# UT-Austin-RPL/FORGE

Measured on AMD Instinct MI355X. Metric: rendered views/sec (5 views, 128^2 px, 64^3 voxel), higher is better.
Workload: dtype f32; 1 GPU; BASELINE configs[1]: FORGE hot path, 1 scene(s)/GPU x 5 input views 256^2 -> 32^3x128 feature grid -> 64^3 render grid -> 5 views x 128^2 rays x 64 samples -> 5 RGB 256^2; HIP rotate, fp32-MFMA implicit-GEMM ResNet-50 trunk / conv1 / ConvGRU (Winograd F(2x2,3x3) x 3 depth taps) / heads / conv_rgb, HIP ray-march (no MIOpen/rocBLAS kernel in the step); eval BN, random-init seeded weights; scenes_per_gpu=1, views_in=5, views_out=5, feature_grid=32, render_grid=64, steps_in_flight=4, launch=hipGraph replay, 4 steps in flight on 4 HIP streams, parallelism=dp1 (scene-sharded, no data-path collective; 4-scalar RCC...

## Files before the change

### forge_amd/csrc/winograd.hip

```cpp
#include "common.h"

namespace forge {

__device__ __forceinline__ float4 add(float4 a, float4 b) { return make_float4(a.x + b.x, a.y + b.y, a.z + b.z, a.w + b.w); }
__device__ __forceinline__ float4 sub(float4 a, float4 b) { return make_float4(a.x - b.x, a.y - b.y, a.z - b.z, a.w - b.w); }
__device__ __forceinline__ float add(float a, float b) { return a + b; }
__device__ __forceinline__ float sub(float a, float b) { return a - b; }
__device__ __forceinline__ float4 fma4(float k, float4 a, float4 b) { return make_float4(fmaf(k, a.x, b.x), fmaf(k, a.y, b.y), fmaf(k, a.z, b.z), fmaf(k, a.w, b.w)); }

__device__ __forceinline__ void f43_six_lines(float p0, float p1, float p2, float p3, float p4, float p5, float& q0, float& q1, float& q2, float& q3, float& q4,
                                              float& q5) {
    const float a02 = p0 - p2, a24 = p2 - p4, s34 = p3 + p4, s12 = p1 + p2, d43 = p4 - p3, d12 = p1 - p2;
    const float d42 = p4 - p2, d31 = p3 - p1, d13 = p1 - p3, d35 = p3 - p5;
    q0 = fmaf(4.f, a02, -a24);
    q1 = fmaf(-4.f, s12, s34);
    q2 = fmaf(4.f, d12, d43);
    q3 = fmaf(2.f, d31, d42);
    q4 = fmaf(-2.f, d31, d42);
    q5 = fmaf(4.f, d13, -d35);
}

__device__ __forceinline__ void tile_decode(long long idx, int per, int cs, int Ht, int Wt, unsigned& r, int& c, int& tw, int& th, unsigned& t) {
    r = (unsigned)(idx / per);
    c = (int)(idx - (long long)r * per) << cs;
    unsigned q = r;
    t = q / (unsigned)Wt;
    tw = (int)(q - t * (unsigned)Wt); q = t; t = q / (unsigned)Ht;
    th = (int)(q - t * (unsigned)Ht);
}

template <typename T>
__device__ __forceinline__ void bt_cols_store(const T (&w)[4], float* vp, int i, long long ptv) {
    *reinterpret_cast<T*>(vp + (4 * i + 0) * ptv) = sub(w[0], w[2]);
    *reinterpret_cast<T*>(vp + (4 * i + 1) * ptv) = add(w[1], w[2]);
    *reinterpret_cast<T*>(vp + (4 * i + 2) * ptv) = sub(w[2], w[1]);
    *reinterpret_cast<T*>(vp + (4 * i + 3) * ptv) = sub(w[1], w[3]);
}

template <typename T, typename I>
__device__ __forceinline__ void bt_d_b_store(const T (&d)[4][4], float* V, I row, int ld, int c, long long ptv) {
    T w[4][4];
#pragma unroll
    for (int j = 0; j < 4; ++j) {
        w[0][j] = sub(d[0][j], d[2][j]);
        w[1][j] = add(d[1][j], d[2][j]);
        w[2][j] = sub(d[2][j], d[1][j]);
        w[3][j] = sub(d[1][j], d[3][j]);
    }
    float* vp = V + (long long)row * ld + c;
#pragma unroll
    for (int i = 0; i < 4; ++i) bt_cols_store(w[i], vp, i, ptv);
}

__device__ __forceinline__ void a_y_at_store(float4 y00, float4 y01, float4 y10, float4 y11, float* mp, long long ptm) {
    const float4 zero = make_float4(0.f, 0.f, 0.f, 0.f);
    const float4 s[4][2] = {{y00, y01}, {add(y00, y10), add(y01, y11)}, {sub(y00, y10), sub(y01, y11)}, {sub(zero, y10), sub(zero, y11)}};
#pragma unroll
    for (int i = 0; i < 4; ++i) {
        *reinterpret_cast<float4*>(mp + (4 * i + 0) * ptm) = s[i][0];
        *reinterpret_cast<float4*>(mp + (4 * i + 1) * ptm) = add(s[i][0], s[i][1]);
        *reinterpret_cast<float4*>(mp + (4 * i + 2) * ptm) = sub(s[i][0], s[i][1]);
        *reinterpret_cast<float4*>(mp + (4 * i + 3) * ptm) = sub(zero, s[i][1]);
    }
}

__device__ __forceinline__ double depth_row_f23(int k, double w0, double w1, double w2) {
    return k == 0 ? w0 : k == 1 ? 0.5 * (w0 + w1 + w2) : k == 2 ? 0.5 * (w0 - w1 + w2) : w2;
}
__device__ __forceinline__ double depth_row_f43(int k, double w0, double w1, double w2) {
    return k == 0 ? 0.25 * w0 : k == 1 ? -((w0 + w2) + w1) / 6.0 : k == 2 ? -((w0 + w2) - w1) / 6.0
         : k == 3 ? ((0.25 * w0 + w2) + 0.5 * w1) / 6.0 : k == 4 ? ((0.25 * w0 + w2) - 0.5 * w1) / 6.0 : w2;
}

template <int NH = 4, double (*HROW)(int, double, double, double) = depth_row_f23>
__device__ __forceinline__ void g_d_gt_store(const double (&d)[3][3], float* up, long long pt) {
    double g[NH][3];
#pragma unroll
    for (int b = 0; b < 3; ++b)
#pragma unroll
        for (int i = 0; i < NH; ++i) g[i][b] = HROW(i, d[0][b], d[1][b], d[2][b]);
#pragma unroll
    for (int i = 0; i < NH; ++i) {
        up[(4 * i + 0) * pt] = (float)g[i][0];
        up[(4 * i + 1) * pt] = (float)(0.5 * (g[i][0] + g[i][1] + g[i][2]));
        up[(4 * i + 2) * pt] = (float)(0.5 * (g[i][0] - g[i][1] + g[i][2]));
        up[(4 * i + 3) * pt] = (float)g[i][2];
    }
}

struct WinoInArgs {
    const float* in; int ld; long long bs;
    float* V; int ldv; long long ptv;
    int n, D, H, W, C;
    int nsum; long long ss;
    float* dM; long long ptm;
};

template <bool DY>
__global__ __launch_bounds__(256) void wino_input_kernel(const WinoInArgs a) {
    const int C4 = a.C >> 2, Ht = a.H >> 1, Wt = a.W >> 1;
    const long long idx = (long long)xcd_remap(blockIdx.x, gridDim.x) * 256 + threadIdx.x;
    const long long R = (long long)a.n * a.D * Ht * Wt;
    if (idx >= R * C4) return;
    unsigned r, t;
    int c, tw, th;
    tile_decode(idx, C4, 2, Ht, Wt, r, c, tw, th, t);
    const unsigned q = t; t = q / (unsigned)a.D;
    const int z = (int)(q - t * (unsigned)a.D);
    const float* base = a.in + ((long long)t * a.bs + (long long)z * a.H * a.W) * a.ld + c;
    float4 d[4][4];
#pragma unroll
    for (int i = 0; i < 4; ++i) {
        const int y = 2 * th - 1 + i;
#pragma unroll
        for (int j = 0; j < 4; ++j) {
            const int x = 2 * tw - 1 + j;
            const bool ok = (unsigned)y < (unsigned)a.H && (unsigned)x < (unsigned)a.W;
            float4 v = make_float4(0.f, 0.f, 0.f, 0.f);
            if (ok) {
                const float* p = base + ((long long)y * a.W + x) * a.ld;
                v = *reinterpret_cast<const float4*>(p);
                if (a.nsum > 1) {
                    for (int k = 1; k < a.nsum; ++k) v = add(v, *reinterpret_cast<const float4*>(p + (long long)k * a.ss * a.ld));
                    const float inv = 1.f / (float)a.nsum;
                    v = make_float4(v.x * inv, v.y * inv, v.z * inv, v.w * inv);
                }
            }
            d[i][j] = v;
        }
    }
    if constexpr (DY) a_y_at_store(d[1][1], d[1][2], d[2][1], d[2][2], a.dM + (long long)r * a.C + c, a.ptm);
    bt_d_b_store(d, a.V, r, a.ldv, c, a.ptv);
}

template <int TH>
__global__ __launch_bounds__(256) void wino_input_dn4_kernel(const WinoInArgs a) {
    constexpr int NR = TH + 2;
    const int Ht = TH == 4 ? a.H >> 2 : a.H >> 1, Wt = a.W >> 1, Dg = a.D >> 2;
    const long long idx = (long long)xcd_remap(blockIdx.x, gridDim.x) * 256 + threadIdx.x;
    const long long RG = (long long)a.n * Dg * Ht * Wt;
    if (idx >= RG * a.C) return;
    unsigned r, t;
    int c, tw, th;
    tile_decode(idx, a.C, 0, Ht, Wt, r, c, tw, th, t);
    const unsigned q = t; t = q / (unsigned)Dg;
    const int g = (int)(q - t * (unsigned)Dg);
    const long long HW = (long long)a.H * a.W;
    const float* base = a.in + (long long)t * a.bs * a.ld + c;
    const float inv = 1.f / (float)a.nsum;
    float d[6][NR][4];
#pragma unroll
    for (int i = 0; i < NR; ++i) {
        const int y = TH * th - 1 + i;
#pragma unroll
        for (int j = 0; j < 4; ++j) {
            const int x = 2 * tw - 1 + j;
            const bool ok = (unsigned)y < (unsigned)a.H && (unsigned)x < (unsigned)a.W;
            float p[6];
#pragma unroll
            for (int e = 0; e < 6; ++e) {
                const int z = 4 * g - 1 + e;
                float v = 0.f;
                if (ok && (unsigned)z < (unsigned)a.D) {
                    const float* s = base + ((long long)z * HW + (long long)y * a.W + x) * a.ld;
                    v = *s;
                    if (a.nsum > 1) {
                        for (int k = 1; k < a.nsum; ++k) v += s[(long long)k * a.ss * a.ld];
                        v *= inv;
                    }
                }
                p[e] = v;
            }
            f43_six_lines(p[0], p[1], p[2], p[3], p[4], p[5], d[0][i][j], d[1][i][j], d[2][i][j], d[3][i][j], d[4][i][j], d[5][i][j]);
        }
    }
    const long long HWt = (long long)Ht * Wt;
    float* vp = a.V + ((((long long)t * Dg + g) * 6) * HWt + (long long)th * Wt + tw) * a.ldv + c;
    if constexpr (TH == 4) {
#pragma unroll
        for (int k = 0; k < 6; ++k) {
#pragma unroll
            for (int j = 0; j < 4; ++j)
                f43_six_lines(d[k][0][j], d[k][1][j], d[k][2][j], d[k][3][j], d[k][4][j], d[k][5][j], d[k][0][j], d[k][1][j], d[k][2][j], d[k][3][j], d[k][4][j], d[k][5][j]);
#pragma unroll
            for (int i = 0; i < 6; ++i) bt_cols_store(d[k][i], vp + k * HWt * a.ldv, i, a.ptv);
        }
    } else {
#pragma unroll
        for (int k = 0; k < 6; ++k) bt_d_b_store(d[k], vp, k * HWt, a.ldv, 0, a.ptv);
    }
}

__global__ __launch_bounds__(256) void wino_weight_kernel(const float* __restrict__ wp, float* __restrict__ U, int Cout, int Cin, int KD, int transpose) {
    const int No = transpose ? Cin : Cout, Nc = transpose ? Cout : Cin;
    const long long idx = (long long)blockIdx.x * 256 + threadIdx.x, per = (long long)No * Nc;
    if (idx >= KD * per) return;
    const int kd = (int)(idx / per);
    const long long oc = idx - kd * per;
    const int o = (int)(oc / Nc), c = (int)(oc - (long long)o * Nc);
    double w[3][3];
#pragma unroll
    for (int a = 0; a < 3; ++a)
#pragma unroll
        for (int b = 0; b < 3; ++b) {
            const int tap = transpose ? ((KD - 1 - kd) * 3 + (2 - a)) * 3 + (2 - b) : (kd * 3 + a) * 3 + b;
            w[a][b] = (double)wp[((long long)tap * Cout + (transpose ? c : o)) * Cin + (transpose ? o : c)];
        }
    g_d_gt_store(w, U + ((long long)kd * No + o) * Nc + c, KD * per);
}

template <int K, double (*ROW)(int, double, double, double), int NH = 4, double (*HROW)(int, double, double, double) = depth_row_f23>
__global__ __launch_bounds__(256) void wino_weight_nest_kernel(const float* __restrict__ wp, float* __restrict__ U, int Cout, int Cin) {
    const long long idx = (long long)blockIdx.x * 256 + threadIdx.x, per = (long long)Cout * Cin;
    if (idx >= per) return;
    double w[3][3][3];
#pragma unroll
    for (int t = 0; t < 27; ++t) w[t / 9][(t / 3) % 3][t % 3] = (double)wp[t * per + idx];
#pragma unroll
    for (int k = 0; k < K; ++k) {
        double d[3][3];
#pragma unroll
        for (int a = 0; a < 3; ++a)
#pragma unroll
            for (int b = 0; b < 3; ++b) d[a][b] = ROW(k, w[0][a][b], w[1][a][b], w[2][a][b]);
        g_d_gt_store<NH, HROW>(d, U + k * per + idx, K * per);
    }
}

enum WinoEpilogue : int { W_BIAS = 0, W_AFFINE_ACT = 1, W_GRU_GATES = 2, W_GRU_OUT = 3 };

struct WinoOutArgs {
    const float* Mm; long long ptm;
    const float* Mm2; long long ptm2, bs2;
    const float* bias; const float* scale; const float* shift; float slope;
    const float* residual;
    const float* aux_h; const float* aux_z;
    float* out; float* out2; float* out3; int ldo;
    int n, D, H, W, Cout, epi;
};

template <int ROWS>
__device__ __forceinline__ void load_planes(float4 (&m)[ROWS][4], const float* Mm, long long ptm, const float* Mm2, long long ptm2, long long bs2, int Cout, unsigned R1, unsigned r, int c) {
    const float* mp = Mm + (long long)r * Cout + c;
#pragma unroll
    for (int i = 0; i < ROWS; ++i)
#pragma unroll
        for (int j = 0; j < 4; ++j) m[i][j] = *reinterpret_cast<const float4*>(mp + (4 * i + j) * ptm);
    if (Mm2) {
        const unsigned nn = r / R1;
        const float* mp2 = Mm2 + ((long long)nn * bs2 + (r - nn * R1)) * Cout + c;
#pragma unroll
        for (int i = 0; i < ROWS; ++i)
#pragma unroll
            for (int j = 0; j < 4; ++j) m[i][j] = add(m[i][j], *reinterpret_cast<const float4*>(mp2 + (4 * i + j) * ptm2));
    }
}

template <int EPI, bool HALF = false, int TH = 2>
__global__ __launch_bounds__(256) void wino_output_kernel(const WinoOutArgs a) {
    static_assert(TH == 2 || (TH == 4 && !HALF), "tiles of 2 x 2 voxels, or of 4 x 2 from the 24 points");
    const int C4 = a.Cout >> 2, Ht = TH == 4 ? a.H >> 2 : a.H >> 1, Wt = a.W >> 1;
    const long long idx = (long long)blockIdx.x * 256 + threadIdx.x;
    const long long R = (long long)a.n * a.D * Ht * Wt;
    if (idx >= R * C4) return;
    unsigned r, t;
    int c, tw, th;
    tile_decode(idx, C4, 2, Ht, Wt, r, c, tw, th, t);
    float4 s[TH][4];
    if constexpr (TH == 4) {
        const float* mp = a.Mm + (long long)r * a.Cout + c;
#pragma unroll
        for (int j = 0; j < 4; ++j) {
            float4 m[6];
#pragma unroll
            for (int i = 0; i < 6; ++i) m[i] = *reinterpret_cast<const float4*>(mp + (4 * i + j) * a.ptm);
            const float4 sl = add(m[1], m[2]), dl = sub(m[1], m[2]), Sl = add(m[3], m[4]), Dl = sub(m[3], m[4]);
            s[0][j] = add(add(sl, Sl), m[0]);
            s[1][j] = fma4(2.f, Dl, dl);
            s[2][j] = fma4(4.f, Sl, sl);
            s[3][j] = add(fma4(8.f, Dl, dl), m[5]);
        }
    } else if constexpr (HALF) {
        load_planes<2>(s, a.Mm, a.ptm, a.Mm2, a.ptm2, a.bs2, a.Cout, (unsigned)(a.D * Ht * Wt), r, c);
    } else {
        float4 m[4][4];
        load_planes<4>(m, a.Mm, a.ptm, a.Mm2, a.ptm2, a.bs2, a.Cout, (unsigned)(a.D * Ht * Wt), r, c);
#pragma unroll
        for (int j = 0; j < 4; ++j) {
            s[0][j] = add(add(m[0][j], m[1][j]), m[2][j]);
            s[1][j] = sub(sub(m[1][j], m[2][j]), m[3][j]);
        }
    }
    float4 y[TH][2];
#pragma unroll
    for (int i = 0; i < TH; ++i) {
        y[i][0] = add(add(s[i][0], s[i][1]), s[i][2]);
        y[i][1] = sub(sub(s[i][1], s[i][2]), s[i][3]);
    }
    float4 bias = make_float4(0.f, 0.f, 0.f, 0.f), sc = make_float4(1.f, 1.f, 1.f, 1.f), sh = bias;
    if (a.bias) bias = *reinterpret_cast<const float4*>(a.bias + c);
    if ((EPI == W_AFFINE_ACT || (EPI == W_GRU_OUT && a.out2)) && a.scale) {
        sc = *reinterpret_cast<const float4*>(a.scale + c);
        sh = *reinterpret_cast<const float4*>(a.shift + c);
    }
    const int Ch = a.Cout >> 1;
    const long long plane = (long long)t * a.H * a.W;
#pragma unroll
    for (int i = 0; i < TH; ++i)
#pragma unroll
        for (int j = 0; j < 2; ++j) {
            const long long orow = plane + (long long)(TH * th + i) * a.W + (2 * tw + j);
            float v[4] = {y[i][j].x + bias.x, y[i][j].y + bias.y, y[i][j].z + bias.z, y[i][j].w + bias.w};
            if (a.residual) {
                const float4 rr = *reinterpret_cast<const float4*>(a.residual + orow * a.Cout + c);
                v[0] += rr.x; v[1] += rr.y; v[2] += rr.z; v[3] += rr.w;
            }
            const float scv[4] = {sc.x, sc.y, sc.z, sc.w}, shv[4] = {sh.x, sh.y, sh.z, sh.w};
            if constexpr (EPI == W_BIAS) {
                *reinterpret_cast<float4*>(a.out + orow * a.ldo + c) = make_float4(v[0], v[1], v[2], v[3]);
            } else if constexpr (EPI == W_AFFINE_ACT) {
#pragma unroll
                for (int k = 0; k < 4; ++k) {
                    const float u = fmaf(v[k], scv[k], shv[k]);
                    v[k] = u > 0.f ? u : u * a.slope;
                }
                *reinterpret_cast<float4*>(a.out + orow * a.ldo + c) = make_float4(v[0], v[1], v[2], v[3]);
            } else if constexpr (EPI == W_GRU_GATES) {
                float g[4];
#pragma unroll
                for (int k = 0; k < 4; ++k) g[k] = 1.f / (1.f + expf(-v[k]));
                if (c < Ch) {
                    *reinterpret_cast<float4*>(a.out + orow * Ch + c) = make_float4(g[0], g[1], g[2], g[3]);
                } else {
                    const float4 h = *reinterpret_cast<const float4*>(a.aux_h + orow * Ch + (c - Ch));
                    *reinterpret_cast<float4*>(a.out2 + orow * Ch + (c - Ch)) = make_float4(h.x * g[0], h.y * g[1], h.z * g[2], h.w * g[3]);
                    if (a.out3) *reinterpret_cast<float4*>(a.out3 + orow * Ch + (c - Ch)) = make_float4(g[0], g[1], g[2], g[3]);
                }
            } else {
                const float4 z4 = *reinterpret_cast<const float4*>(a.aux_z + orow * a.Cout + c);
                const float4 h4 = *reinterpret_cast<const float4*>(a.aux_h + orow * a.Cout + c);
                const float zv[4] = {z4.x, z4.y, z4.z, z4.w}, hv[4] = {h4.x, h4.y, h4.z, h4.w};
                float cand[4], hn[4];
#pragma unroll
                for (int k = 0; k < 4; ++k) {
                    cand[k] = tanhf(v[k]);
                    hn[k] = hv[k] * (1.f - zv[k]) + cand[k] * zv[k];
                }
                *reinterpret_cast<float4*>(a.out + orow * a.ldo + c) = make_float4(hn[0], hn[1], hn[2], hn[3]);
                if (a.out2)
                    *reinterpret_cast<float4*>(a.out2 + orow * a.ldo + c) =
                        make_float4(fmaf(hn[0], scv[0], shv[0]), fmaf(hn[1], scv[1], shv[1]), fmaf(hn[2], scv[2], shv[2]), fmaf(hn[3], scv[3], shv[3]));
                if (a.out3) *reinterpret_cast<float4*>(a.out3 + orow * a.ldo + c) = make_float4(cand[0], cand[1], cand[2], cand[3]);
            }
        }
}

struct WinoDyArgs {
    const float* dy; int ldy;
    float* dM; long long ptm;
    int n, D, H, W, Cout;
};

__global__ __launch_bounds__(256) void wino_dy_kernel(const WinoDyArgs a) {
    const int C4 = a.Cout >> 2, Ht = a.H >> 1, Wt = a.W >> 1;
    const long long idx = (long long)blockIdx.x * 256 + threadIdx.x;
    const long long R = (long long)a.n * a.D * Ht * Wt;
    if (idx >= R * C4) return;
    unsigned r, t;
    int c, tw, th;
    tile_decode(idx, C4, 2, Ht, Wt, r, c, tw, th, t);
    const float* yp = a.dy + ((long long)t * a.H * a.W + (long long)(2 * th) * a.W + 2 * tw) * a.ldy + c;
    float4 y[2][2];
#pragma unroll
    for (int i = 0; i < 2; ++i)
#pragma unroll
        for (int j = 0; j < 2; ++j) y[i][j] = *reinterpret_cast<const float4*>(yp + ((long long)i * a.W + j) * a.ldy);
    a_y_at_store(y[0][0], y[0][1], y[1][0], y[1][1], a.dM + (long long)r * a.Cout + c, a.ptm);
}

__global__ __launch_bounds__(256) void wino_dw_kernel(const float* __restrict__ dU, float* __restrict__ dw, int Cout, int Cin, int KD) {
    const long long idx = (long long)blockIdx.x * 256 + threadIdx.x, per = (long long)Cout * Cin;
    if (idx >= KD * per) return;
    const int kd = (int)(idx / per);
    const long long oc = idx - kd * per;
    const long long pt = KD * per;
    float u[4][4];
#pragma unroll
    for (int i = 0; i < 4; ++i)
#pragma unroll
        for (int j = 0; j < 4; ++j) u[i][j] = dU[(4 * i + j) * pt + kd * per + oc];
    float g[3][4];
#pragma unroll
    for (int j = 0; j < 4; ++j) {
        g[0][j] = u[0][j] + 0.5f * (u[1][j] + u[2][j]);
        g[1][j] = 0.5f * (u[1][j] - u[2][j]);
        g[2][j] = 0.5f * (u[1][j] + u[2][j]) + u[3][j];
    }
#pragma unroll
    for (int a_ = 0; a_ < 3; ++a_) {
        float* o = dw + ((long long)((kd * 3 + a_) * 3) * per) + oc;
        o[0 * per] += g[a_][0] + 0.5f * (g[a_][1] + g[a_][2]);
        o[1 * per] += 0.5f * (g[a_][1] - g[a_][2]);
        o[2 * per] += 0.5f * (g[a_][1] + g[a_][2]) + g[a_][3];
    }
}

}

using namespace forge;

extern "C" int forge_wino_dy(const float* dy, int ldy, float* dM, int n, int D, int H, int W, int Cout, forge_stream_t stream) {
    FORGE_REQUIRE(dy && dM, FORGE_EINVAL, "forge_wino_dy: null pointer argument");
    FORGE_REQUIRE(n > 0 && D > 0 && H > 0 && W > 0 && H % 2 == 0 && W % 2 == 0 && Cout > 0 && Cout % 4 == 0 && ldy >= Cout && ldy % 4 == 0, FORGE_ESHAPE,
                  "forge_wino_dy: n=%d D=%d H=%d W=%d Cout=%d ldy=%d (H, W even; Cout, ldy multiples of 4)", n, D, H, W, Cout, ldy);
    WinoDyArgs a;
    const long long R = (long long)n * D * (H / 2) * (W / 2);
    a.dy = dy; a.ldy = ldy; a.dM = dM; a.ptm = R * Cout; a.n = n; a.D = D; a.H = H; a.W = W; a.Cout = Cout;
    FORGE_REQUIRE(R < (1ll << 31), FORGE_ESHAPE, "forge_wino_dy: more than 2^31 tiles; split the batch");
    const long long total = R * (Cout / 4), grid = (total + 255) / 256;
    FORGE_REQUIRE(grid < (1ll << 31), FORGE_ESHAPE, "forge_wino_dy: grid too large");
    hipLaunchKernelGGL(wino_dy_kernel, dim3((unsigned)grid), dim3(256), 0, (hipStream_t)stream, a);
    FORGE_LAUNCH_CHECK("forge_wino_dy");
    return 0;
}

extern "C" int forge_wino_dw(const float* dU, float* dw, int Cout, int Cin, int kd, forge_stream_t stream) {
    FORGE_REQUIRE(dU && dw && Cout > 0 && Cin > 0 && (kd == 1 || kd == 3), FORGE_EINVAL, "forge_wino_dw: bad argument (kd = 1 or 3)");
    const long long total = (long long)kd * Cout * Cin;
    hipLaunchKernelGGL(wino_dw_kernel, dim3((unsigned)((total + 255) / 256)), dim3(256), 0, (hipStream_t)stream, dU, dw, Cout, Cin, kd);
    FORGE_LAUNCH_CHECK("forge_wino_dw");
    return 0;
}

template <typename K, typename... A>
static int wino_weights_launch(const char* name, K kernel, long long total, forge_stream_t stream, A... args) {
    hipLaunchKernelGGL(kernel, dim3((unsigned)((total + 255) / 256)), dim3(256), 0, (hipStream_t)stream, args...);
    FORGE_LAUNCH_CHECK(name);
    return 0;
}

extern "C" int forge_wino_weights(const float* wp, float* U, int Cout, int Cin, int kd, int transpose, forge_stream_t stream) {
    FORGE_REQUIRE(wp && U && Cout > 0 && Cin > 0 && (kd == 1 || kd == 3), FORGE_EINVAL, "forge_wino_weights: bad argument (kd = 1 or 3)");
    return wino_weights_launch("forge_wino_weights", wino_weight_kernel, (long long)kd * Cout * Cin, stream, wp, U, Cout, Cin, kd, transpose);
}

extern "C" int forge_wino_weights_dn(const float* wp, float* Ud, int Cout, int Cin, forge_stream_t stream) {
    FORGE_REQUIRE(wp && Ud && Cout > 0 && Cin > 0, FORGE_EINVAL, "forge_wino_weights_dn: bad argument");
    return wino_weights_launch("forge_wino_weights_dn", wino_weight_nest_kernel<4, depth_row_f23>, (long long)Cout * Cin, stream, wp, Ud, Cout, Cin);
}

extern "C" int forge_wino_weights_dn4(const float* wp, float* Ud, int Cout, int Cin, forge_stream_t stream) {
    FORGE_REQUIRE(wp && Ud && Cout > 0 && Cin > 0, FORGE_EINVAL, "forge_wino_weights_dn4: bad argument");
    return wino_weights_launch("forge_wino_weights_dn4", wino_weight_nest_kernel<6, depth_row_f43>, (long long)Cout * Cin, stream, wp, Ud, Cout, Cin);
}

extern "C" int forge_wino_weights_dn4h(const float* wp, float* Ud, int Cout, int Cin, forge_stream_t stream) {
    FORGE_REQUIRE(wp && Ud && Cout > 0 && Cin > 0, FORGE_EINVAL, "forge_wino_weights_dn4h: bad argument");
    return wino_weights_launch("forge_wino_weights_dn4h", wino_weight_nest_kernel<6, depth_row_f43, 6, depth_row_f43>, (long long)Cout * Cin, stream, wp, Ud, Cout, Cin);
}

enum WinoInKind { IN_PLAIN, IN_DN4, IN_DY, IN_DN4H };

static int wino_input_impl(const char* name, WinoInKind kind, const float* in, int ld, long long bs, float* V, int ldv, long long ptv, float* dM, int n, int D, int H,
                           int W, int C, int nsum, long long sum_stride, forge_stream_t stream) {
    const bool dn4 = kind == IN_DN4 || kind == IN_DN4H;
    const int th = kind == IN_DN4H ? 4 : 2;
    FORGE_REQUIRE(in && V && (kind != IN_DY || dM), FORGE_EINVAL, "%s: null pointer argument", name);
    FORGE_REQUIRE(nsum >= 1 && (nsum == 1 || sum_stride > 0), FORGE_EINVAL, "%s: nsum >= 1, and a positive sum_stride (rows) with nsum > 1", name);
    FORGE_REQUIRE(!dn4 || (D > 0 && D % 4 == 0), FORGE_EINVAL, "%s: D=%d must be a multiple of 4", name, D);
    FORGE_REQUIRE(kind != IN_DN4H || (D >= 8 && H > 0 && H % 4 == 0), FORGE_EINVAL, "%s: D=%d H=%d (D >= 8; H a multiple of 4)", name, D, H);
    const bool ok = n > 0 && D > 0 && H > 0 && W > 0 && H % 2 == 0 && W % 2 == 0 && C > 0 && C % 4 == 0 && ld >= C && ld % 4 == 0 && ldv >= C && ldv % 4 == 0;
    if (kind == IN_DY)
        FORGE_REQUIRE(ok, FORGE_ESHAPE, "%s: n=%d D=%d H=%d W=%d C=%d ld=%d (H, W even; C, ld multiples of 4)", name, n, D, H, W, C, ld);
    FORGE_REQUIRE(ok, FORGE_ESHAPE, "%s: n=%d D=%d H=%d W=%d C=%d ld=%d ldv=%d (H, W even; C, ld, ldv multiples of 4)", name, n, D, H, W, C, ld, ldv);
    WinoInArgs a;
    a.in = in; a.ld = ld; a.bs = bs > 0 ? bs : (long long)D * H * W; a.V = V; a.ldv = ldv; a.n = n; a.D = D; a.H = H; a.W = W; a.C = C;
    a.nsum = nsum; a.ss = sum_stride;
    const long long R = (long long)n * (dn4 ? D / 4 : D) * (H / th) * (W / 2), rows = dn4 ? 6 * R : R;
    a.ptv = ptv > 0 ? ptv : rows * ldv;
    a.dM = dM; a.ptm = dM ? R * C : 0;
    FORGE_REQUIRE(rows < (1ll << 31), FORGE_ESHAPE, dn4 ? "%s: more than 2^31 operand rows; split the batch" : "%s: more than 2^31 tiles; split the batch", name);
    const long long total = R * (dn4 ? C : C / 4), grid = (total + 255) / 256;
    FORGE_REQUIRE(grid < (1ll << 31), FORGE_ESHAPE, "%s: grid too large", name);
    const dim3 g((unsigned)grid), b(256);
    if (kind == IN_DN4H) hipLaunchKernelGGL(wino_input_dn4_kernel<4>, g, b, 0, (hipStream_t)stream, a);
    else if (dn4) hipLaunchKernelGGL(wino_input_dn4_kernel<2>, g, b, 0, (hipStream_t)stream, a);
    else if (kind == IN_DY) hipLaunchKernelGGL(wino_input_kernel<true>, g, b, 0, (hipStream_t)stream, a);
    else hipLaunchKernelGGL(wino_input_kernel<false>, g, b, 0, (hipStream_t)stream, a);
    FORGE_LAUNCH_CHECK(name);
    return 0;
}

extern "C" int forge_wino_input(const float* in, int ld, long long bs, float* V, int ldv, long long ptv, int n, int D, int H, int W, int C,
                                int nsum, long long sum_stride, forge_stream_t stream) {
    return wino_input_impl("forge_wino_input", IN_PLAIN, in, ld, bs, V, ldv, ptv, nullptr, n, D, H, W, C, nsum, sum_stride, stream);
}

extern "C" int forge_wino_input_dn4(const float* in, int ld, long long bs, float* V6, int ldv, long long ptv, int n, int D, int H, int W, int C,
                                    int nsum, long long sum_stride, forge_stream_t stream) {
    return wino_input_impl("forge_wino_input_dn4", IN_DN4, in, ld, bs, V6, ldv, ptv, nullptr, n, D, H, W, C, nsum, sum_stride, stream);
}

extern "C" int forge_wino_input_dn4h(const float* in, int ld, long long bs, float* V, int ldv, long long ptv, int n, int D, int H, int W, int C,
                                     int nsum, long long sum_stride, forge_stream_t stream) {
    return wino_input_impl("forge_wino_input_dn4h", IN_DN4H, in, ld, bs, V, ldv, ptv, nullptr, n, D, H, W, C, nsum, sum_stride, stream);
}

extern "C" int forge_wino_input_dy(const float* dy, int ld, float* V, float* dM, int n, int D, int H, int W, int C, forge_stream_t stream) {
    return wino_input_impl("forge_wino_input_dy", IN_DY, dy, ld, 0, V, C, 0, dM, n, D, H, W, C, 1, 0, stream);
}

static int wino_output_impl(const float* Mm, const float* Mm2, long long bs2, long long pt2, const float* bias, const float* scale, const float* shift, float slope, const float* residual,
                            const float* aux_h, const float* aux_z, float* out, float* out2, float* out3, int n, int D, int H, int W, int Cout,
                            int ldo, int epilogue, bool half, forge_stream_t stream) {
    FORGE_REQUIRE(Mm && out, FORGE_EINVAL, "forge_wino_output: null pointer argument");
    FORGE_REQUIRE(n > 0 && D > 0 && H > 0 && W > 0 && H % 2 == 0 && W % 2 == 0 && Cout > 0 && Cout % 8 == 0 && ldo % 4 == 0, FORGE_ESHAPE,
                  "forge_wino_output: n=%d D=%d H=%d W=%d Cout=%d ldo=%d (H, W even; Cout multiple of 8; ldo of 4)", n, D, H, W, Cout, ldo);
    FORGE_REQUIRE(epilogue >= 0 && epilogue <= 3, FORGE_EINVAL, "forge_wino_output: unknown epilogue %d", epilogue);
    FORGE_REQUIRE(epilogue == W_GRU_GATES ? ldo == Cout / 2 : ldo >= Cout, FORGE_ESHAPE,
                  "forge_wino_output: ldo=%d (epilogues 0, 1, 3: ldo >= Cout=%d; epilogue 2: ldo == Cout / 2)", ldo, Cout);
    FORGE_REQUIRE(epilogue != W_AFFINE_ACT || (scale && shift), FORGE_EINVAL, "forge_wino_output: affine epilogue needs scale/shift");
    FORGE_REQUIRE(epilogue != W_GRU_GATES || (aux_h && out2), FORGE_EINVAL, "forge_wino_output: GRU gate epilogue needs aux_h, out2");
    FORGE_REQUIRE(epilogue != W_GRU_OUT || (aux_h && aux_z && (!out2 || (scale && shift))), FORGE_EINVAL,
                  "forge_wino_output: GRU out epilogue needs aux_h, aux_z (and scale/shift with out2)");
    FORGE_REQUIRE(out3 == nullptr || epilogue == W_GRU_GATES || epilogue == W_GRU_OUT, FORGE_EINVAL, "forge_wino_output: out3 is a GRU-epilogue output");
    WinoOutArgs a;
    const long long R = (long long)n * D * (H / 2) * (W / 2);
    a.Mm = Mm; a.ptm = R * Cout; a.Mm2 = Mm2; a.bs2 = bs2 > 0 ? bs2 : (long long)D * (H / 2) * (W / 2); a.ptm2 = pt2 > 0 ? pt2 : R * Cout; a.bias = bias; a.scale = scale; a.shift = shift; a.slope = slope; a.residual = residual; a.aux_h = aux_h; a.aux_z = aux_z;
    a.out = out; a.out2 = out2; a.out3 = out3; a.ldo = ldo; a.n = n; a.D = D; a.H = H; a.W = W; a.Cout = Cout; a.epi = epilogue;
    FORGE_REQUIRE(R < (1ll << 31), FORGE_ESHAPE, "forge_wino_output: more than 2^31 tiles; split the batch");
    const long long total = R * (Cout / 4), grid = (total + 255) / 256;
    FORGE_REQUIRE(grid < (1ll << 31), FORGE_ESHAPE, "forge_wino_output: grid too large");
    const dim3 g((unsigned)grid), b(256);
    hipStream_t st = (hipStream_t)stream;
    if (half) {
        switch (epilogue) {
            case W_BIAS: hipLaunchKernelGGL((wino_output_kernel<W_BIAS, true>), g, b, 0, st, a); break;
            case W_AFFINE_ACT: hipLaunchKernelGGL((wino_output_kernel<W_AFFINE_ACT, true>), g, b, 0, st, a); break;
            case W_GRU_GATES: hipLaunchKernelGGL((wino_output_kernel<W_GRU_GATES, true>), g, b, 0, st, a); break;
            default: hipLaunchKernelGGL((wino_output_kernel<W_GRU_OUT, true>), g, b, 0, st, a); break;
        }
    } else {
        switch (epilogue) {
            case W_BIAS: hipLaunchKernelGGL(wino_output_kernel<W_BIAS>, g, b, 0, st, a); break;
            case W_AFFINE_ACT: hipLaunchKernelGGL(wino_output_kernel<W_AFFINE_ACT>, g, b, 0, st, a); break;
            case W_GRU_GATES: hipLaunchKernelGGL(wino_output_kernel<W_GRU_GATES>, g, b, 0, st, a); break;
            default: hipLaunchKernelGGL(wino_output_kernel<W_GRU_OUT>, g, b, 0, st, a); break;
        }
    }
    FORGE_LAUNCH_CHECK("forge_wino_output");
    return 0;
}

extern "C" int forge_wino_output(const float* Mm, const float* Mm2, long long bs2, long long pt2, const float* bias, const float* scale, const float* shift, float slope, const float* residual,
                                 const float* aux_h, const float* aux_z, float* out, float* out2, float* out3, int n, int D, int H, int W, int Cout,
                                 int ldo, int epilogue, forge_stream_t stream) {
    return wino_output_impl(Mm, Mm2, bs2, pt2, bias, scale, shift, slope, residual, aux_h, aux_z, out, out2, out3, n, D, H, W, Cout, ldo, epilogue, false, stream);
}

extern "C" int forge_wino_output_half(const float* Mm8, const float* Mm2_8, long long bs2, long long pt2, const float* bias, const float* scale, const float* shift, float slope,
                                      const float* residual, const float* aux_h, const float* aux_z, float* out, float* out2, float* out3, int n, int D, int H, int W,
                                      int Cout, int ldo, int epilogue, forge_stream_t stream) {
    return wino_output_impl(Mm8, Mm2_8, bs2, pt2, bias, scale, shift, slope, residual, aux_h, aux_z, out, out2, out3, n, D, H, W, Cout, ldo, epilogue, true, stream);
}

extern "C" int forge_wino_output_dn4h(const float* Mm, const float* bias, const float* scale, const float* shift, const float* aux_h, const float* aux_z, float* out,
                                      float* out2, float* out3, int n, int D, int H, int W, int Cout, int ldo, int epilogue, forge_stream_t stream) {
    FORGE_REQUIRE(Mm && out && aux_h, FORGE_EINVAL, "forge_wino_output_dn4h: null pointer argument");
    FORGE_REQUIRE(n > 0 && D > 0 && H > 0 && W > 0 && H % 4 == 0 && W % 2 == 0 && Cout > 0 && Cout % 8 == 0 && ldo % 4 == 0, FORGE_ESHAPE,
                  "forge_wino_output_dn4h: n=%d D=%d H=%d W=%d Cout=%d ldo=%d (H multiple of 4, W even; Cout multiple of 8; ldo of 4)", n, D, H, W, Cout, ldo);
    FORGE_REQUIRE(epilogue == W_GRU_GATES || epilogue == W_GRU_OUT, FORGE_EINVAL, "forge_wino_output_dn4h: epilogue %d is not a GRU tail (2, 3)", epilogue);
    FORGE_REQUIRE(epilogue == W_GRU_GATES ? ldo == Cout / 2 : ldo >= Cout, FORGE_ESHAPE,
                  "forge_wino_output_dn4h: ldo=%d (epilogue 3: ldo >= Cout=%d; epilogue 2: ldo == Cout / 2)", ldo, Cout);
    FORGE_REQUIRE(epilogue != W_GRU_GATES || out2, FORGE_EINVAL, "forge_wino_output_dn4h: GRU gate epilogue needs out2");
    FORGE_REQUIRE(epilogue != W_GRU_OUT || (aux_z && (!out2 || (scale && shift))), FORGE_EINVAL,
                  "forge_wino_output_dn4h: GRU out epilogue needs aux_z (and scale/shift with out2)");
    WinoOutArgs a;
    const long long R = (long long)n * D * (H / 4) * (W / 2);
    a.Mm = Mm; a.ptm = R * Cout; a.Mm2 = nullptr; a.bs2 = 0; a.ptm2 = 0; a.bias = bias; a.scale = scale; a.shift = shift; a.slope = 1.f; a.residual = nullptr;
    a.aux_h = aux_h; a.aux_z = aux_z; a.out = out; a.out2 = out2; a.out3 = out3; a.ldo = ldo; a.n = n; a.D = D; a.H = H; a.W = W; a.Cout = Cout; a.epi = epilogue;
    FORGE_REQUIRE(R < (1ll << 31), FORGE_ESHAPE, "forge_wino_output_dn4h: more than 2^31 tiles; split the batch");
    const long long total = R * (Cout / 4), grid = (total + 255) / 256;
    FORGE_REQUIRE(grid < (1ll << 31), FORGE_ESHAPE, "forge_wino_output_dn4h: grid too large");
    const dim3 g((unsigned)grid), b(256);
    if (epilogue == W_GRU_GATES) hipLaunchKernelGGL((wino_output_kernel<W_GRU_GATES, false, 4>), g, b, 0, (hipStream_t)stream, a);
    else hipLaunchKernelGGL((wino_output_kernel<W_GRU_OUT, false, 4>), g, b, 0, (hipStream_t)stream, a);
    FORGE_LAUNCH_CHECK("forge_wino_output_dn4h");
    return 0;
}
```

Measured before the change: 1048 views/s.

## Restructure Winograd depth-input kernel per wave and narrow output channel vectors

The depth-4 input transform now maps one wave to one tile with 64 channels across lanes. Tile coordinates and base addresses become wave-uniform through readfirstlane, so address arithmetic moves to scalar registers. The 4-row variant streams its column transforms in pairs instead of holding the full 6x6x4 array, which cuts register pressure, and it adds an occupancy hint. The mean-over-views path becomes a compile-time template. The output transform now handles 2 channels per thread for the dn4h and unhalved affine epilogues, giving more threads and fewer live registers at the cost of narrower memory accesses.

```diff
diff --git a/forge_amd/csrc/winograd.hip b/forge_amd/csrc/winograd.hip
--- a/forge_amd/csrc/winograd.hip
+++ b/forge_amd/csrc/winograd.hip
@@ -7,6 +7,21 @@
 __device__ __forceinline__ float add(float a, float b) { return a + b; }
 __device__ __forceinline__ float sub(float a, float b) { return a - b; }
 __device__ __forceinline__ float4 fma4(float k, float4 a, float4 b) { return make_float4(fmaf(k, a.x, b.x), fmaf(k, a.y, b.y), fmaf(k, a.z, b.z), fmaf(k, a.w, b.w)); }
+__device__ __forceinline__ float2 add(float2 a, float2 b) { return make_float2(a.x + b.x, a.y + b.y); }
+__device__ __forceinline__ float2 sub(float2 a, float2 b) { return make_float2(a.x - b.x, a.y - b.y); }
+__device__ __forceinline__ float2 fma4(float k, float2 a, float2 b) { return make_float2(fmaf(k, a.x, b.x), fmaf(k, a.y, b.y)); }
+__device__ __forceinline__ float fma4(float k, float a, float b) { return fmaf(k, a, b); }
+
+template <int N> struct chan_vec;
+template <> struct chan_vec<1> { using type = float; };
+template <> struct chan_vec<2> { using type = float2; };
+template <> struct chan_vec<4> { using type = float4; };
+__device__ __forceinline__ void lanes(float v, float (&o)[1]) { o[0] = v; }
+__device__ __forceinline__ void lanes(float2 v, float (&o)[2]) { o[0] = v.x; o[1] = v.y; }
+__device__ __forceinline__ void lanes(float4 v, float (&o)[4]) { o[0] = v.x; o[1] = v.y; o[2] = v.z; o[3] = v.w; }
+__device__ __forceinline__ float pack(const float (&v)[1]) { return v[0]; }
+__device__ __forceinline__ float2 pack(const float (&v)[2]) { return make_float2(v[0], v[1]); }
+__device__ __forceinline__ float4 pack(const float (&v)[4]) { return make_float4(v[0], v[1], v[2], v[3]); }
 
 __device__ __forceinline__ void f43_six_lines(float p0, float p1, float p2, float p3, float p4, float p5, float& q0, float& q1, float& q2, float& q3, float& q4,
                                               float& q5) {
@@ -133,61 +148,118 @@
     bt_d_b_store(d, a.V, r, a.ldv, c, a.ptv);
 }
 
-template <int TH>
-__global__ __launch_bounds__(256) void wino_input_dn4_kernel(const WinoInArgs a) {
+
+template <int NR>
+struct Dn4Patch { long long org, sz, sy, sx, sv; bool okz[6], oky[NR], okx[4]; };
+
+typedef __attribute__((address_space(1))) char wave_gchar;
+typedef __attribute__((address_space(1))) float wave_gfloat;
+__device__ __forceinline__ wave_gfloat* wave_elem(const void* p, unsigned cb) {
+    const unsigned long long u = reinterpret_cast<unsigned long long>(p);
+    const unsigned lo = __builtin_amdgcn_readfirstlane((unsigned)u), hi = __builtin_amdgcn_readfirstlane((unsigned)(u >> 32));
+    return (wave_gfloat*)((wave_gchar*)(((unsigned long long)hi << 32) | lo) + cb);
+}
+
+template <bool MEAN, int NR>
+__device__ __forceinline__ void dn4_depth_elem(const WinoInArgs& a, const Dn4Patch<NR>& pt, unsigned cb, float inv, int i, int j, float& q0, float& q1, float& q2,
+                                               float& q3, float& q4, float& q5) {
+    const bool ok = pt.oky[i] && pt.okx[j];
+    float p[6];
+#pragma unroll
+    for (int e = 0; e < 6; ++e) {
+        float v = 0.f;
+        if (ok && pt.okz[e]) {
+            const char* s = reinterpret_cast<const char*>(a.in) + (pt.org + (e * pt.sz + i * pt.sy + j * pt.sx));
+            v = *wave_elem(s, cb);
+            if constexpr (MEAN) {
+                for (int k = 1; k < a.nsum; ++k) v += *wave_elem(s + k * pt.sv, cb);
+                v *= inv;
+            }
+        }
+        p[e] = v;
+    }
+    f43_six_lines(p[0], p[1], p[2], p[3], p[4], p[5], q0, q1, q2, q3, q4, q5);
+}
+
+template <bool MEAN>
+__device__ __forceinline__ void dn4h_depth_col(const WinoInArgs& a, const Dn4Patch<6>& pt, unsigned cb, float inv, int j, float (&q)[6][6]) {
+#pragma unroll
+    for (int i = 0; i < 6; ++i) dn4_depth_elem<MEAN>(a, pt, cb, inv, i, j, q[0][i], q[1][i], q[2][i], q[3][i], q[4][i], q[5][i]);
+}
+
+__device__ __forceinline__ void dn4h_rows(float (&q)[6][6]) {
+#pragma unroll
+    for (int k = 0; k < 6; ++k) f43_six_lines(q[k][0], q[k][1], q[k][2], q[k][3], q[k][4], q[k][5], q[k][0], q[k][1], q[k][2], q[k][3], q[k][4], q[k][5]);
+}
+
+__device__ __forceinline__ void store_at(float* u, unsigned cb, float v) { *wave_elem(u, cb) = v; }
+
+template <int TH, bool MEAN>
+__global__ __launch_bounds__(256, TH == 4 ? 5 : 1) void wino_input_dn4_kernel(const WinoInArgs a) {
     constexpr int NR = TH + 2;
     const int Ht = TH == 4 ? a.H >> 2 : a.H >> 1, Wt = a.W >> 1, Dg = a.D >> 2;
-    const long long idx = (long long)xcd_remap(blockIdx.x, gridDim.x) * 256 + threadIdx.x;
+    const int cw = (a.C + 63) >> 6;
+    const long long wv = (long long)xcd_remap(blockIdx.x, gridDim.x) * 4 + __builtin_amdgcn_readfirstlane((int)(threadIdx.x >> 6));
     const long long RG = (long long)a.n * Dg * Ht * Wt;
-    if (idx >= RG * a.C) return;
+    if (wv >= RG * cw) return;
     unsigned r, t;
     int c, tw, th;
-    tile_decode(idx, a.C, 0, Ht, Wt, r, c, tw, th, t);
+    tile_decode(wv, cw, 6, Ht, Wt, r, c, tw, th, t);
+    c += (int)(threadIdx.x & 63);
+    if (c >= a.C) return;
+    const unsigned cb = (unsigned)c << 2;
     const unsigned q = t; t = q / (unsigned)Dg;
-    const int g = (int)(q - t * (unsigned)Dg);
+    const int g = __builtin_amdgcn_readfirstlane((int)(q - t * (unsigned)Dg));
+    t = (unsigned)__builtin_amdgcn_readfirstlane((int)t);
+    th = __builtin_amdgcn_readfirstlane(th); tw = __builtin_amdgcn_readfirstlane(tw);
+    Dn4Patch<NR> pt;
+    const int z0 = 4 * g - 1, y0 = TH * th - 1, x0 = 2 * tw - 1;
     const long long HW = (long long)a.H * a.W;
-    const float* base = a.in + (long long)t * a.bs * a.ld + c;
+    pt.sx = 4ll * a.ld; pt.sy = pt.sx * a.W; pt.sz = pt.sx * HW; pt.sv = pt.sx * a.ss;
+    pt.org = ((long long)t * a.bs + (long long)z0 * HW + (long long)y0 * a.W + x0) * pt.sx;
+#pragma unroll
+    for (int e = 0; e < 6; ++e) pt.okz[e] = (unsigned)(z0 + e) < (unsigned)a.D;
+#pragma unroll
+    for (int i = 0; i < NR; ++i) pt.oky[i] = (unsigned)(y0 + i) < (unsigned)a.H;
+#pragma unroll
+    for (int j = 0; j < 4; ++j) pt.okx[j] = (unsigned)(x0 + j) < (unsigned)a.W;
     const float inv = 1.f / (float)a.nsum;
-    float d[6][NR][4];
-#pragma unroll
-    for (int i = 0; i < NR; ++i) {
-        const int y = TH * th - 1 + i;
-#pragma unroll
-        for (int j = 0; j < 4; ++j) {
-            const int x = 2 * tw - 1 + j;
-            const bool ok = (unsigned)y < (unsigned)a.H && (unsigned)x < (unsigned)a.W;
-            float p[6];
-#pragma unroll
-            for (int e = 0; e < 6; ++e) {
-                const int z = 4 * g - 1 + e;
-                float v = 0.f;
-                if (ok && (unsigned)z < (unsigned)a.D) {
-                    const float* s = base + ((long long)z * HW + (long long)y * a.W + x) * a.ld;
-                    v = *s;
-                    if (a.nsum > 1) {
-                        for (int k = 1; k < a.nsum; ++k) v += s[(long long)k * a.ss * a.ld];
-                        v *= inv;
-                    }
-                }
-                p[e] = v;
+    const long long HWt = (long long)Ht * Wt;
+    float* vp = a.V + ((((long long)t * Dg + g) * 6) * HWt + (long long)th * Wt + tw) * a.ldv;
+    if constexpr (TH == 4) {
+        const long long pk = HWt * a.ldv;
+        float wa[6][6], wb[6][6];
+        dn4h_depth_col<MEAN>(a, pt, cb, inv, 2, wb);
+        dn4h_rows(wb);
+        dn4h_depth_col<MEAN>(a, pt, cb, inv, 0, wa);
+        dn4h_rows(wa);
+#pragma unroll
+        for (int k = 0; k < 6; ++k)
+#pragma unroll
+            for (int i = 0; i < 6; ++i) store_at(vp + k * pk + (4 * i + 0) * a.ptv, cb, sub(wa[k][i], wb[k][i]));
+        dn4h_depth_col<MEAN>(a, pt, cb, inv, 1, wa);
+        dn4h_rows(wa);
+#pragma unroll
+        for (int k = 0; k < 6; ++k)
+#pragma unroll
+            for (int i = 0; i < 6; ++i) {
+                store_at(vp + k * pk + (4 * i + 1) * a.ptv, cb, add(wa[k][i], wb[k][i]));
+                store_at(vp + k * pk + (4 * i + 2) * a.ptv, cb, sub(wb[k][i], wa[k][i]));
             }
-            f43_six_lines(p[0], p[1], p[2], p[3], p[4], p[5], d[0][i][j], d[1][i][j], d[2][i][j], d[3][i][j], d[4][i][j], d[5][i][j]);
-        }
-    }
-    const long long HWt = (long long)Ht * Wt;
-    float* vp = a.V + ((((long long)t * Dg + g) * 6) * HWt + (long long)th * Wt + tw) * a.ldv + c;
-    if constexpr (TH == 4) {
-#pragma unroll
-        for (int k = 0; k < 6; ++k) {
-#pragma unroll
-            for (int j = 0; j < 4; ++j)
-                f43_six_lines(d[k][0][j], d[k][1][j], d[k][2][j], d[k][3][j], d[k][4][j], d[k][5][j], d[k][0][j], d[k][1][j], d[k][2][j], d[k][3][j], d[k][4][j], d[k][5][j]);
-#pragma unroll
-            for (int i = 0; i < 6; ++i) bt_cols_store(d[k][i], vp + k * HWt * a.ldv, i, a.ptv);
-        }
+        dn4h_depth_col<MEAN>(a, pt, cb, inv, 3, wb);
+        dn4h_rows(wb);
+#pragma unroll
+        for (int k = 0; k < 6; ++k)
+#pragma unroll
+            for (int i = 0; i < 6; ++i) store_at(vp + k * pk + (4 * i + 3) * a.ptv, cb, sub(wa[k][i], wb[k][i]));
     } else {
-#pragma unroll
-        for (int k = 0; k < 6; ++k) bt_d_b_store(d[k], vp, k * HWt, a.ldv, 0, a.ptv);
+        float d[6][NR][4];
+#pragma unroll
+        for (int i = 0; i < NR; ++i)
+#pragma unroll
+            for (int j = 0; j < 4; ++j) dn4_depth_elem<MEAN>(a, pt, cb, inv, i, j, d[0][i][j], d[1][i][j], d[2][i][j], d[3][i][j], d[4][i][j], d[5][i][j]);
+#pragma unroll
+        for (int k = 0; k < 6; ++k) bt_d_b_store(d[k], vp, k * HWt, a.ldv, c, a.ptv);
     }
 }
 
@@ -239,42 +311,46 @@
     int n, D, H, W, Cout, epi;
 };
 
-template <int ROWS>
-__device__ __forceinline__ void load_planes(float4 (&m)[ROWS][4], const float* Mm, long long ptm, const float* Mm2, long long ptm2, long long bs2, int Cout, unsigned R1, unsigned r, int c) {
+template <int ROWS, typename T>
+__device__ __forceinline__ void load_planes(T (&m)[ROWS][4], const float* Mm, long long ptm, const float* Mm2, long long ptm2, long long bs2, int Cout, unsigned R1, unsigned r, int c) {
     const float* mp = Mm + (long long)r * Cout + c;
 #pragma unroll
     for (int i = 0; i < ROWS; ++i)
 #pragma unroll
-        for (int j = 0; j < 4; ++j) m[i][j] = *reinterpret_cast<const float4*>(mp + (4 * i + j) * ptm);
+        for (int j = 0; j < 4; ++j) m[i][j] = *reinterpret_cast<const T*>(mp + (4 * i + j) * ptm);
     if (Mm2) {
         const unsigned nn = r / R1;
         const float* mp2 = Mm2 + ((long long)nn * bs2 + (r - nn * R1)) * Cout + c;
 #pragma unroll
         for (int i = 0; i < ROWS; ++i)
 #pragma unroll
-            for (int j = 0; j < 4; ++j) m[i][j] = add(m[i][j], *reinterpret_cast<const float4*>(mp2 + (4 * i + j) * ptm2));
-    }
-}
-
-template <int EPI, bool HALF = false, int TH = 2>
+            for (int j = 0; j < 4; ++j) m[i][j] = add(m[i][j], *reinterpret_cast<const T*>(mp2 + (4 * i + j) * ptm2));
+    }
+}
+
+__host__ __device__ constexpr int wino_out_cpt(int epi, bool half, int th) { return th == 4 || (epi == 1 && !half) ? 2 : 4; }
+
+template <int EPI, bool HALF = false, int TH = 2, int CPT = wino_out_cpt(EPI, HALF, TH)>
 __global__ __launch_bounds__(256) void wino_output_kernel(const WinoOutArgs a) {
     static_assert(TH == 2 || (TH == 4 && !HALF), "tiles of 2 x 2 voxels, or of 4 x 2 from the 24 points");
-    const int C4 = a.Cout >> 2, Ht = TH == 4 ? a.H >> 2 : a.H >> 1, Wt = a.W >> 1;
+    static_assert(CPT == 1 || CPT == 2 || CPT == 4, "channels per thread: float, float2 or float4");
+    using V = typename chan_vec<CPT>::type;
+    const int Cp = a.Cout / CPT, Ht = TH == 4 ? a.H >> 2 : a.H >> 1, Wt = a.W >> 1;
     const long long idx = (long long)blockIdx.x * 256 + threadIdx.x;
     const long long R = (long long)a.n * a.D * Ht * Wt;
-    if (idx >= R * C4) return;
+    if (idx >= R * Cp) return;
     unsigned r, t;
     int c, tw, th;
-    tile_decode(idx, C4, 2, Ht, Wt, r, c, tw, th, t);
-    float4 s[TH][4];
+    tile_decode(idx, Cp, CPT == 4 ? 2 : CPT == 2 ? 1 : 0, Ht, Wt, r, c, tw, th, t);
+    V s[TH][4];
     if constexpr (TH == 4) {
         const float* mp = a.Mm + (long long)r * a.Cout + c;
 #pragma unroll
         for (int j = 0; j < 4; ++j) {
-            float4 m[6];
-#pragma unroll
-            for (int i = 0; i < 6; ++i) m[i] = *reinterpret_cast<const float4*>(mp + (4 * i + j) * a.ptm);
-            const float4 sl = add(m[1], m[2]), dl = sub(m[1], m[2]), Sl = add(m[3], m[4]), Dl = sub(m[3], m[4]);
+            V m[6];
+#pragma unroll
+            for (int i = 0; i < 6; ++i) m[i] = *reinterpret_cast<const V*>(mp + (4 * i + j) * a.ptm);
+            const V sl = add(m[1], m[2]), dl = sub(m[1], m[2]), Sl = add(m[3], m[4]), Dl = sub(m[3], m[4]);
             s[0][j] = add(add(sl, Sl), m[0]);
             s[1][j] = fma4(2.f, Dl, dl);
             s[2][j] = fma4(4.f, Sl, sl);
@@ -283,7 +359,7 @@
     } else if constexpr (HALF) {
         load_planes<2>(s, a.Mm, a.ptm, a.Mm2, a.ptm2, a.bs2, a.Cout, (unsigned)(a.D * Ht * Wt), r, c);
     } else {
-        float4 m[4][4];
+        V m[4][4];
         load_planes<4>(m, a.Mm, a.ptm, a.Mm2, a.ptm2, a.bs2, a.Cout, (unsigned)(a.D * Ht * Wt), r, c);
 #pragma unroll
         for (int j = 0; j < 4; ++j) {
@@ -291,17 +367,19 @@
             s[1][j] = sub(sub(m[1][j], m[2][j]), m[3][j]);
         }
     }
-    float4 y[TH][2];
+    V y[TH][2];
 #pragma unroll
     for (int i = 0; i < TH; ++i) {
         y[i][0] = add(add(s[i][0], s[i][1]), s[i][2]);
         y[i][1] = sub(sub(s[i][1], s[i][2]), s[i][3]);
     }
-    float4 bias = make_float4(0.f, 0.f, 0.f, 0.f), sc = make_float4(1.f, 1.f, 1.f, 1.f), sh = bias;
-    if (a.bias) bias = *reinterpret_cast<const float4*>(a.bias + c);
+    float bias[CPT], scv[CPT], shv[CPT];
+#pragma unroll
+    for (int k = 0; k < CPT; ++k) bias[k] = 0.f, scv[k] = 1.f, shv[k] = 0.f;
+    if (a.bias) lanes(*reinterpret_cast<const V*>(a.bias + c), bias);
     if ((EPI == W_AFFINE_ACT || (EPI == W_GRU_OUT && a.out2)) && a.scale) {
-        sc = *reinterpret_cast<const float4*>(a.scale + c);
-        sh = *reinterpret_cast<const float4*>(a.shift + c);
+        lanes(*reinterpret_cast<const V*>(a.scale + c), scv);
+        lanes(*reinterpret_cast<const V*>(a.shift + c), shv);
     }
     const int Ch = a.Cout >> 1;
     const long long plane = (long long)t * a.H * a.W;
@@ -310,47 +388,56 @@
 #pragma unroll
         for (int j = 0; j < 2; ++j) {
             const long long orow = plane + (long long)(TH * th + i) * a.W + (2 * tw + j);
-            float v[4] = {y[i][j].x + bias.x, y[i][j].y + bias.y, y[i][j].z + bias.z, y[i][j].w + bias.w};
+            float v[CPT];
+            lanes(y[i][j], v);
+#pragma unroll
+            for (int k = 0; k < CPT; ++k) v[k] = v[k] + bias[k];
             if (a.residual) {
-                const float4 rr = *reinterpret_cast<const float4*>(a.residual + orow * a.Cout + c);
-                v[0] += rr.x; v[1] += rr.y; v[2] += rr.z; v[3] += rr.w;
+                float rr[CPT];
+                lanes(*reinterpret_cast<const V*>(a.residual + orow * a.Cout + c), rr);
+#pragma unroll
+                for (int k = 0; k < CPT; ++k) v[k] += rr[k];
             }
-            const float scv[4] = {sc.x, sc.y, sc.z, sc.w}, shv[4] = {sh.x, sh.y, sh.z, sh.w};
             if constexpr (EPI == W_BIAS) {
-                *reinterpret_cast<float4*>(a.out + orow * a.ldo + c) = make_float4(v[0], v[1], v[2], v[3]);
+                *reinterpret_cast<V*>(a.out + orow * a.ldo + c) = pack(v);
             } else if constexpr (EPI == W_AFFINE_ACT) {
 #pragma unroll
-                for (int k = 0; k < 4; ++k) {
+                for (int k = 0; k < CPT; ++k) {
                     const float u = fmaf(v[k], scv[k], shv[k]);
                     v[k] = u > 0.f ? u : u * a.slope;
                 }
-                *reinterpret_cast<float4*>(a.out + orow * a.ldo + c) = make_float4(v[0], v[1], v[2], v[3]);
+                *reinterpret_cast<V*>(a.out + orow * a.ldo + c) = pack(v);
             } else if constexpr (EPI == W_GRU_GATES) {
-                float g[4];
-#pragma unroll
-                for (int k = 0; k < 4; ++k) g[k] = 1.f / (1.f + expf(-v[k]));
+                float g[CPT];
+#pragma unroll
+                for (int k = 0; k < CPT; ++k) g[k] = 1.f / (1.f + expf(-v[k]));
                 if (c < Ch) {
-                    *reinterpret_cast<float4*>(a.out + orow * Ch + c) = make_float4(g[0], g[1], g[2], g[3]);
+                    *reinterpret_cast<V*>(a.out + orow * Ch + c) = pack(g);
                 } else {
-                    const float4 h = *reinterpret_cast<const float4*>(a.aux_h + orow * Ch + (c - Ch));
-                    *reinterpret_cast<float4*>(a.out2 + orow * Ch + (c - Ch)) = make_float4(h.x * g[0], h.y * g[1], h.z * g[2], h.w * g[3]);
-                    if (a.out3) *reinterpret_cast<float4*>(a.out3 + orow * Ch + (c - Ch)) = make_float4(g[0], g[1], g[2], g[3]);
+                    float h[CPT], hg[CPT];
+                    lanes(*reinterpret_cast<const V*>(a.aux_h + orow * Ch + (c - Ch)), h);
+#pragma unroll
+                    for (int k = 0; k < CPT; ++k) hg[k] = h[k] * g[k];
+                    *reinterpret_cast<V*>(a.out2 + orow * Ch + (c - Ch)) = pack(hg);
+                    if (a.out3) *reinterpret_cast<V*>(a.out3 + orow * Ch + (c - Ch)) = pack(g);
                 }
             } else {
-                const float4 z4 = *reinterpret_cast<const float4*>(a.aux_z + orow * a.Cout + c);
-                const float4 h4 = *reinterpret_cast<const float4*>(a.aux_h + orow * a.Cout + c);
-                const float zv[4] = {z4.x, z4.y, z4.z, z4.w}, hv[4] = {h4.x, h4.y, h4.z, h4.w};
-                float cand[4], hn[4];
-#pragma unroll
-                for (int k = 0; k < 4; ++k) {
+                float zv[CPT], hv[CPT], cand[CPT], hn[CPT];
+                lanes(*reinterpret_cast<const V*>(a.aux_z + orow * a.Cout + c), zv);
+                lanes(*reinterpret_cast<const V*>(a.aux_h + orow * a.Cout + c), hv);
+#pragma unroll
+                for (int k = 0; k < CPT; ++k) {
                     cand[k] = tanhf(v[k]);
                     hn[k] = hv[k] * (1.f - zv[k]) + cand[k] * zv[k];
                 }
-                *reinterpret_cast<float4*>(a.out + orow * a.ldo + c) = make_float4(hn[0], hn[1], hn[2], hn[3]);
-                if (a.out2)
-                    *reinterpret_cast<float4*>(a.out2 + orow * a.ldo + c) =
-                        make_float4(fmaf(hn[0], scv[0], shv[0]), fmaf(hn[1], scv[1], shv[1]), fmaf(hn[2], scv[2], shv[2]), fmaf(hn[3], scv[3], shv[3]));
-                if (a.out3) *reinterpret_cast<float4*>(a.out3 + orow * a.ldo + c) = make_float4(cand[0], cand[1], cand[2], cand[3]);
+                *reinterpret_cast<V*>(a.out + orow * a.ldo + c) = pack(hn);
+                if (a.out2) {
+                    float ha[CPT];
+#pragma unroll
+                    for (int k = 0; k < CPT; ++k) ha[k] = fmaf(hn[k], scv[k], shv[k]);
+                    *reinterpret_cast<V*>(a.out2 + orow * a.ldo + c) = pack(ha);
+                }
+                if (a.out3) *reinterpret_cast<V*>(a.out3 + orow * a.ldo + c) = pack(cand);
             }
         }
 }
@@ -480,11 +567,13 @@
     a.ptv = ptv > 0 ? ptv : rows * ldv;
     a.dM = dM; a.ptm = dM ? R * C : 0;
     FORGE_REQUIRE(rows < (1ll << 31), FORGE_ESHAPE, dn4 ? "%s: more than 2^31 operand rows; split the batch" : "%s: more than 2^31 tiles; split the batch", name);
-    const long long total = R * (dn4 ? C : C / 4), grid = (total + 255) / 256;
+    const long long total = dn4 ? R * ((C + 63) / 64) * 64 : R * (C / 4), grid = (total + 255) / 256;
     FORGE_REQUIRE(grid < (1ll << 31), FORGE_ESHAPE, "%s: grid too large", name);
     const dim3 g((unsigned)grid), b(256);
-    if (kind == IN_DN4H) hipLaunchKernelGGL(wino_input_dn4_kernel<4>, g, b, 0, (hipStream_t)stream, a);
-    else if (dn4) hipLaunchKernelGGL(wino_input_dn4_kernel<2>, g, b, 0, (hipStream_t)stream, a);
+    if (kind == IN_DN4H && nsum > 1) hipLaunchKernelGGL((wino_input_dn4_kernel<4, true>), g, b, 0, (hipStream_t)stream, a);
+    else if (kind == IN_DN4H) hipLaunchKernelGGL((wino_input_dn4_kernel<4, false>), g, b, 0, (hipStream_t)stream, a);
+    else if (dn4 && nsum > 1) hipLaunchKernelGGL((wino_input_dn4_kernel<2, true>), g, b, 0, (hipStream_t)stream, a);
+    else if (dn4) hipLaunchKernelGGL((wino_input_dn4_kernel<2, false>), g, b, 0, (hipStream_t)stream, a);
     else if (kind == IN_DY) hipLaunchKernelGGL(wino_input_kernel<true>, g, b, 0, (hipStream_t)stream, a);
     else hipLaunchKernelGGL(wino_input_kernel<false>, g, b, 0, (hipStream_t)stream, a);
     FORGE_LAUNCH_CHECK(name);
@@ -529,7 +618,7 @@
     a.Mm = Mm; a.ptm = R * Cout; a.Mm2 = Mm2; a.bs2 = bs2 > 0 ? bs2 : (long long)D * (H / 2) * (W / 2); a.ptm2 = pt2 > 0 ? pt2 : R * Cout; a.bias = bias; a.scale = scale; a.shift = shift; a.slope = slope; a.residual = residual; a.aux_h = aux_h; a.aux_z = aux_z;
     a.out = out; a.out2 = out2; a.out3 = out3; a.ldo = ldo; a.n = n; a.D = D; a.H = H; a.W = W; a.Cout = Cout; a.epi = epilogue;
     FORGE_REQUIRE(R < (1ll << 31), FORGE_ESHAPE, "forge_wino_output: more than 2^31 tiles; split the batch");
-    const long long total = R * (Cout / 4), grid = (total + 255) / 256;
+    const long long total = R * (Cout / wino_out_cpt(epilogue, half, 2)), grid = (total + 255) / 256;
     FORGE_REQUIRE(grid < (1ll << 31), FORGE_ESHAPE, "forge_wino_output: grid too large");
     const dim3 g((unsigned)grid), b(256);
     hipStream_t st = (hipStream_t)stream;
@@ -580,7 +669,7 @@
     a.Mm = Mm; a.ptm = R * Cout; a.Mm2 = nullptr; a.bs2 = 0; a.ptm2 = 0; a.bias = bias; a.scale = scale; a.shift = shift; a.slope = 1.f; a.residual = nullptr;
     a.aux_h = aux_h; a.aux_z = aux_z; a.out = out; a.out2 = out2; a.out3 = out3; a.ldo = ldo; a.n = n; a.D = D; a.H = H; a.W = W; a.Cout = Cout; a.epi = epilogue;
     FORGE_REQUIRE(R < (1ll << 31), FORGE_ESHAPE, "forge_wino_output_dn4h: more than 2^31 tiles; split the batch");
-    const long long total = R * (Cout / 4), grid = (total + 255) / 256;
+    const long long total = R * (Cout / wino_out_cpt(epilogue, false, 4)), grid = (total + 255) / 256;
     FORGE_REQUIRE(grid < (1ll << 31), FORGE_ESHAPE, "forge_wino_output_dn4h: grid too large");
     const dim3 g((unsigned)grid), b(256);
     if (epilogue == W_GRU_GATES) hipLaunchKernelGGL((wino_output_kernel<W_GRU_GATES, false, 4>), g, b, 0, (hipStream_t)stream, a);
```

After: 1038 views/s. 1.0% lower.
